# jixinya/EAMM

Hardware: AMD Instinct MI355X
Metric: 256x256 frames/sec (dense-motion + generator forward) (higher is better)
Workload: dtype f32; 1 GPU; 256x256, 10 keypoints, batch=16 synthetic frames per GPU per step, source encoded once per clip (BASELINE.json configs[2]); parallelism=frame-sharded x1

## Files before the change

eamm_amd/csrc/conv_winograd4.hip:

```cpp
#include "conv_common.h"

#include <algorithm>
#include <cstdlib>

namespace eamm {

typedef __attribute__((address_space(3))) void* lds_ptr_t;
typedef float f32x4_t __attribute__((ext_vector_type(4)));

template <int VEC> struct vec_of;
template <> struct vec_of<1> { typedef float type; };
template <> struct vec_of<2> { typedef float type __attribute__((ext_vector_type(2))); };
template <> struct vec_of<4> { typedef float type __attribute__((ext_vector_type(4))); };

template <typename T> __device__ __forceinline__ T vfma(float a, T x, T y);
template <> __device__ __forceinline__ float vfma<float>(float a, float x, float y) { return fmaf(a, x, y); }
template <> __device__ __forceinline__ vec_of<2>::type vfma(float a, vec_of<2>::type x, vec_of<2>::type y) {
    vec_of<2>::type r;
    r[0] = fmaf(a, x[0], y[0]); r[1] = fmaf(a, x[1], y[1]);
    return r;
}
template <> __device__ __forceinline__ vec_of<4>::type vfma(float a, vec_of<4>::type x, vec_of<4>::type y) {
    vec_of<4>::type r;
    r[0] = fmaf(a, x[0], y[0]); r[1] = fmaf(a, x[1], y[1]); r[2] = fmaf(a, x[2], y[2]); r[3] = fmaf(a, x[3], y[3]);
// ... 38 lines not shown
    const size_t total = Mq * cvn;
    const size_t bid = (by_xcd & 1) ? (size_t)xcd_remap((int)blockIdx.x, (int)gridDim.x) : (size_t)blockIdx.x;
    for (size_t idx = bid * blockDim.x + threadIdx.x; idx < total; idx += (size_t)gridDim.x * blockDim.x) {
        const int cv = (int)(idx % cvn);
        const size_t q = idx / cvn;
        const int qx = (int)(q % Wq);
        const int qy = (int)((q / Wq) % Hq);
        const int b = (int)(q / ((size_t)Wq * Hq));
        T sc = T(1.f), sh = T(0.f);
        if (s != nullptr) {
            sc = reinterpret_cast<const T*>(s)[cv];
            sh = reinterpret_cast<const T*>(t)[cv];
        }
        const T* img = reinterpret_cast<const T*>(x) + (size_t)b * H * W * cvn + cv;
        T d[6][6];
        int yo[6], xo[6];
        bool oky[6], okx[6];
#pragma unroll
        for (int i = 0; i < 6; ++i) {
            const int yy = 4 * qy - 1 + i, xx = 4 * qx - 1 + i;
            oky[i] = (unsigned)yy < (unsigned)H;
            okx[i] = (unsigned)xx < (unsigned)W;
            yo[i] = min(max(yy, 0), H - 1) * W;
            xo[i] = min(max(xx, 0), W - 1);
        }
#pragma unroll
        for (int i = 0; i < 6; ++i)
#pragma unroll
            for (int j = 0; j < 6; ++j) d[i][j] = img[(size_t)(yo[i] + xo[j]) * cvn];
#pragma unroll
        for (int i = 0; i < 6; ++i)
#pragma unroll
            for (int j = 0; j < 6; ++j) {
                T v = d[i][j];
                if (s != nullptr) v = vrelu_affine(v, sc, sh);
                d[i][j] = (oky[i] && okx[j]) ? v : T(0.f);
            }
#pragma unroll
        for (int j = 0; j < 6; ++j) bt6(d[0][j], d[1][j], d[2][j], d[3][j], d[4][j], d[5][j]);
        T* out = reinterpret_cast<T*>(V) + q * cvn + cv;
        const size_t plane = Mq * cvn;
#pragma unroll
        for (int i = 0; i < 6; ++i) {
            bt6(d[i][0], d[i][1], d[i][2], d[i][3], d[i][4], d[i][5]);
            if constexpr (VEC == 4) {
                if (by_xcd & 2) {
                    const __amdgpu_buffer_rsrc_t rs = __builtin_amdgcn_make_buffer_rsrc((void*)V, 0, (unsigned)(36 * plane * 16), 0x00020000);
#pragma unroll
                    for (int j = 0; j < 6; ++j)
                        __builtin_amdgcn_raw_buffer_store_b128(__builtin_bit_cast(u32x4, d[i][j]), rs,
                                                               (unsigned)(((size_t)(i * 6 + j) * plane + q * cvn + cv) * 16), 0, 2);
                    continue;
                }
            }
#pragma unroll
            for (int j = 0; j < 6; ++j) out[(size_t)(i * 6 + j) * plane] = d[i][j];
        }
    }
}

struct Wino4Args {
    const float* V;
    const float* U;
    const float* bias;
    unsigned v_bytes, u_bytes;
    int Mq, C, Cout;
    int H, W;
    int mtiles, ntiles;
    int act;
    const float* resid;
    float* out;
    int groups;
    float* zout;
    float* epi_scratch;
};

__constant__ float WINO4_AT[4][8] = {{1.f, 1.f, 1.f, 1.f, 1.f, 0.f, 0.f, 0.f},
                                     {0.f, 1.f, -1.f, 2.f, -2.f, 0.f, 0.f, 0.f},
                                     {0.f, 1.f, 1.f, 4.f, 4.f, 0.f, 0.f, 0.f},
                                     {0.f, 1.f, -1.f, 8.f, -8.f, 1.f, 0.f, 0.f}};

template <int NT, int WM, int WN, int SUB, int NST, int PE, int DBG = 0>
__global__ __launch_bounds__(WM* WN * 64) void wino4_gemm_kernel(const Wino4Args p) {
    constexpr int NW = WM * WN, NTHR = NW * 64;
    constexpr int BM = WM * 16, BN = WN * NT * 16, BK = CONV_BK;
    constexpr int A_STAGE = SUB * BM * BK, B_STAGE = SUB * BN * BK;
    constexpr int A_INSTR = BM / 8 / NW, B_INSTR = BN / 8 / NW;
    constexpr int NPIECE = SUB * (A_INSTR + B_INSTR);
    constexpr bool TRACE = DBG == 8 || DBG == 9;
    static_assert(BM % (8 * NW) == 0 && BN % (8 * NW) == 0, "tile rows must split evenly over the waves");
    static_assert(BK == 32, "two 16-wide K steps per chunk");

    extern __shared__ __attribute__((aligned(16))) float smem[];
    float* const As = smem;
    float* const Bs = smem + NST * A_STAGE;

    const int tid = threadIdx.x;
    const int lane = tid & 63;
    const int wave = __builtin_amdgcn_readfirstlane(tid >> 6);
    const int r16 = lane & 15, g = lane >> 4;
    const int wm = wave / WN, wn = wave % WN;

    const int L = xcd_remap(blockIdx.x, gridDim.x);
    const int ntile = L % p.ntiles;
    const int mtile = (L / p.ntiles) % p.mtiles;
    const int grp = L / (p.ntiles * p.mtiles);
    const int xis_per = 36 / p.groups;
    const int xi0 = grp * xis_per;
    const int mbase = mtile * BM;
    const int cchunks = p.C / BK;
    const int ci_base = xi0 * cchunks;
    const int nsuper = xis_per * cchunks / SUB;

    unsigned arow_off[A_INSTR];
#pragma unroll
    for (int j = 0; j < A_INSTR; ++j) {
        const int row = (wave * A_INSTR + j) * 8 + (lane >> 3);
        const int slot = (lane & 7) ^ ((row >> 1) & 7);
        const int m = mbase + row;
        arow_off[j] = m < p.Mq ? (unsigned)(m * p.C + slot * 4) * 4u : 0xFFFFF000u;
    }
    const unsigned b_lane = (unsigned)lane * 16u;
    const __amdgpu_buffer_rsrc_t rsv = __builtin_amdgcn_make_buffer_rsrc((void*)p.V, 0, p.v_bytes, 0x00020000);
    const __amdgpu_buffer_rsrc_t rsu = __builtin_amdgcn_make_buffer_rsrc((void*)p.U, 0, p.u_bytes, 0x00020000);
    const unsigned plane_bytes = (unsigned)p.Mq * (unsigned)p.C * 4u;
    const unsigned a_wrap = plane_bytes - (unsigned)(cchunks * BK * 4);

    unsigned sa_off = (unsigned)xi0 * plane_bytes;
    unsigned sb_off = (unsigned)((ntile * 36 * cchunks + ci_base) * BN * BK) * 4u +
                      (unsigned)(wave * B_INSTR * 8 * BK) * 4u;
    int dma_cc = 0, n_st = 0;
    auto dma_advance = [&]() {
        dma_cc += SUB;
        sa_off += SUB * BK * 4;
        if (dma_cc == cchunks) {
            dma_cc = 0;
            sa_off += a_wrap;
        }
        sb_off += SUB * BN * BK * 4;
        n_st = n_st + 1 == NST ? 0 : n_st + 1;
    };
    auto dma_piece = [&](auto kc) {
        constexpr int k = decltype(kc)::value;
        constexpr int sub = k / (A_INSTR + B_INSTR), r = k % (A_INSTR + B_INSTR);
        if constexpr (r < A_INSTR) {
            float* dst = As + n_st * A_STAGE + sub * (BM * BK) + (wave * A_INSTR + r) * (8 * BK) - sub * BK;
            const unsigned vo = arow_off[r];
            __builtin_amdgcn_raw_ptr_buffer_load_lds(rsv, (lds_ptr_t)dst, 16, vo, sa_off, sub * BK * 4, DBG == 40 ? 2 : 0);
        } else {
            constexpr int j = r - A_INSTR;
            float* dst = Bs + n_st * B_STAGE + sub * (BN * BK) + (wave * B_INSTR + j) * (8 * BK);
            __builtin_amdgcn_raw_ptr_buffer_load_lds(rsu, (lds_ptr_t)dst, 16, b_lane,
                                                     sb_off + (unsigned)((sub * BN + j * 8) * BK * 4), 0, 0);
        }
    };

    f32x4_t acc[NT];
    f32x4_t Z[4][NT];
    f32x4_t Y[16][NT];
    static_for<NT>([&](auto jc) {
        constexpr int j = decltype(jc)::value;
        static_for<4>([&](auto rc) {
            constexpr int r = decltype(rc)::value;
            acc[j][r] = 0.f;
            static_for<4>([&](auto qc) { Z[decltype(qc)::value][j][r] = 0.f; });
            static_for<16>([&](auto pc) { Y[decltype(pc)::value][j][r] = 0.f; });
        });
    });

    const int sw = (r16 >> 1) & 7;
    constexpr int STEPS = SUB * 2;
    constexpr int MF = 4 * NT;
    constexpr int TOTAL_MF = STEPS * MF;
    static_assert(PE >= 1 && NPIECE * PE <= TOTAL_MF, "DMA pieces must fit in the interval");
    auto compute = [&](int st, auto more_c, auto young_c) {
        constexpr bool MORE = decltype(more_c)::value && DBG != 1 && DBG != 9, YOUNG = decltype(young_c)::value;
        f32x4_t a[2], b[2][NT];
        auto fetch = [&](int step, int buf) {
            const int sub = step >> 1, s = step & 1;
            const int slot = ((4 * s + g) ^ sw) << 2;
            const float* a_base = As + st * A_STAGE + sub * (BM * BK) + (wm * 16 + r16) * BK + slot;
            const float* b_base = Bs + st * B_STAGE + sub * (BN * BK) + (wn * NT * 16 + r16) * BK + slot;
            a[buf] = *reinterpret_cast<const f32x4_t*>(a_base);
#pragma unroll
            for (int j = 0; j < NT; ++j) b[buf][j] = *reinterpret_cast<const f32x4_t*>(b_base + j * 16 * BK);
        };
        fetch(0, 0);
        if constexpr (MORE && YOUNG) static_for<NPIECE>([&](auto kc) { dma_piece(kc); });
        static_for<STEPS>([&](auto sc) {
            constexpr int step = decltype(sc)::value;
            if constexpr (step + 1 < STEPS) fetch(step + 1, (step + 1) & 1);
            __builtin_amdgcn_sched_barrier(0);
            static_for<MF>([&](auto qc) {
                constexpr int q = decltype(qc)::value;
                constexpr int t = q / NT, j = q % NT;
                acc[j] = __builtin_amdgcn_mfma_f32_16x16x4f32(a[step & 1][t], b[step & 1][j][t], acc[j], 0, 0, 0);
                constexpr int gi = step * MF + q;
                if constexpr (MORE && !YOUNG && gi % PE == PE - 1 && gi / PE < NPIECE) {
                    __builtin_amdgcn_sched_barrier(0);
                    dma_piece(std::integral_constant<int, gi / PE>{});
                    __builtin_amdgcn_sched_barrier(0);
                }
            });
        });
    };
    const bool young = wave >= NW / 2;
    auto interval = [&](int st, bool more) {
        if (more) {
            if (young) compute(st, std::true_type{}, std::true_type{});
            else compute(st, std::true_type{}, std::false_type{});
            dma_advance();
        } else {
            compute(st, std::false_type{}, std::false_type{});
        }
    };

    auto fold_x = [&](int j) {
        const float c0 = WINO4_AT[0][j], c1 = WINO4_AT[1][j], c2 = WINO4_AT[2][j], c3 = WINO4_AT[3][j];
        static_for<NT>([&](auto jc) {
            constexpr int jj = decltype(jc)::value;
            static_for<4>([&](auto rc) {
                constexpr int r = decltype(rc)::value;
                const float m = acc[jj][r];
                Z[0][jj][r] = fmaf(c0, m, Z[0][jj][r]);
                Z[1][jj][r] = fmaf(c1, m, Z[1][jj][r]);
                Z[2][jj][r] = fmaf(c2, m, Z[2][jj][r]);
                Z[3][jj][r] = fmaf(c3, m, Z[3][jj][r]);
                acc[jj][r] = 0.f;
            });
        });
    };
    auto fold_y = [&](int i) {
        const float c0 = WINO4_AT[0][i], c1 = WINO4_AT[1][i], c2 = WINO4_AT[2][i], c3 = WINO4_AT[3][i];
        static_for<NT>([&](auto jc) {
            constexpr int jj = decltype(jc)::value;
            static_for<4>([&](auto qc) {
                constexpr int q = decltype(qc)::value;
                static_for<4>([&](auto rc) {
                    constexpr int r = decltype(rc)::value;
                    const float z = Z[q][jj][r];
                    Y[0 + q][jj][r] = fmaf(c0, z, Y[0 + q][jj][r]);
                    Y[4 + q][jj][r] = fmaf(c1, z, Y[4 + q][jj][r]);
                    Y[8 + q][jj][r] = fmaf(c2, z, Y[8 + q][jj][r]);
                    Y[12 + q][jj][r] = fmaf(c3, z, Y[12 + q][jj][r]);
                    Z[q][jj][r] = 0.f;
                });
            });
        });
    };

    auto store_z = [&](int i) {
        static_for<4>([&](auto qc) {
            constexpr int q = decltype(qc)::value;
            static_for<NT>([&](auto jc) {
                constexpr int jj = decltype(jc)::value;
                const int col = ntile * BN + wn * NT * 16 + jj * 16 + r16;
                static_for<4>([&](auto rc) {
                    constexpr int r = decltype(rc)::value;
                    const int row = mbase + wm * 16 + 4 * g + r;
                    if (row < p.Mq && col < p.Cout) p.zout[((size_t)(i * 4 + q) * p.Mq + row) * p.Cout + col] = Z[q][jj][r];
                    Z[q][jj][r] = 0.f;
                });
            });
        });
    };

    constexpr int D = NST - 1;
    const int per_xi = cchunks / SUB;
    for (int k = 0; k < D && k < nsuper; ++k) {
        static_for<NPIECE>([&](auto kc) { dma_piece(kc); });
        dma_advance();
    }
    if (D > 1 && nsuper >= D) {
        asm volatile("s_waitcnt vmcnt(%0)" ::"n"((D - 1) * NPIECE) : "memory");
    } else {
        asm volatile("s_waitcnt vmcnt(0)" ::: "memory");
    }
    __syncthreads();
    int st = 0;
    int xi_left = per_xi, xj = xi0 % 6, xrow = xi0 / 6;
    const bool half_rows = p.groups == 12;
    for (int sc = 0; sc < nsuper; ++sc) {
        const bool more = sc + D < nsuper;
        long long ts0 = 0, ts1 = 0, ts2 = 0;
        if constexpr (TRACE) ts0 = __builtin_readcyclecounter();
        interval(st, more);
        if constexpr (TRACE) ts1 = __builtin_readcyclecounter();
        if (--xi_left == 0) {
            xi_left = per_xi;
            fold_x(xj);
            if (++xj == 6) {
                xj = 0;
                if (p.zout != nullptr)
                    store_z(half_rows ? grp : xrow++);
                else
                    fold_y(xrow++);
            }
        }
        if constexpr (TRACE) ts2 = __builtin_readcyclecounter();
        if (D > 1 && more) {
            asm volatile("s_waitcnt vmcnt(%0)" ::"n"((D - 1) * NPIECE) : "memory");
        } else {
            asm volatile("s_waitcnt vmcnt(0)" ::: "memory");
        }
        if constexpr (TRACE) {
            const long long ts3 = __builtin_readcyclecounter();
            if (blockIdx.x == 0 && lane == 0 && sc < 72) {
                long long* dbg = reinterpret_cast<long long*>(const_cast<float*>(p.resid)) + (wave * 72 + sc) * 4;
                dbg[0] = ts0; dbg[1] = ts1; dbg[2] = ts2; dbg[3] = ts3;
            }
        }
        __syncthreads();
        st = st + 1 == NST ? 0 : st + 1;
    }

    if (p.zout != nullptr) {
        if (half_rows && xj != 0) store_z(grp);
        return;
    }
    constexpr int LDO = BN + 4, C4 = BN / 4, RPP = NTHR / (4 * C4), PER = BM / RPP;
    static_assert(NTHR % (4 * C4) == 0 && BM % RPP == 0, "tile must split evenly over the threads");
    const int Hq = p.H >> 2, Wq = p.W >> 2;
    float bias[NT];
#pragma unroll
    for (int j = 0; j < NT; ++j) bias[j] = p.bias[ntile * BN + wn * NT * 16 + j * 16 + r16];
    const int e_c4 = tid % C4, e_px = (tid / C4) & 3, e_row0 = tid / (4 * C4);
    const int e_n = ntile * BN + e_c4 * 4;
    unsigned e_off[PER];
#pragma unroll
    for (int k = 0; k < PER; ++k) {
        const int m = mbase + e_row0 + k * RPP;
        const int qx = m % Wq, tq = m / Wq;
        const int qy = tq % Hq, bb = tq / Hq;
        const unsigned o = (unsigned)(((bb * p.H + 4 * qy) * p.W + 4 * qx + e_px) * p.Cout + e_n) * 4u;
        e_off[k] = (m < p.Mq && e_n < p.Cout) ? o : 0xFFFFFFF0u;
    }
    const unsigned out_bytes = (unsigned)p.Mq * 16u * (unsigned)p.Cout * 4u;
    const __amdgpu_buffer_rsrc_t rso = __builtin_amdgcn_make_buffer_rsrc((void*)p.out, 0, out_bytes, 0x00020000);
    const __amdgpu_buffer_rsrc_t rsr =
        __builtin_amdgcn_make_buffer_rsrc((void*)p.resid, 0, (p.resid != nullptr && !TRACE) ? out_bytes : 0u, 0x00020000);
    const float lo = p.act == ACT_RELU ? 0.f : -INFINITY;
    const unsigned row_bytes = (unsigned)p.W * (unsigned)p.Cout * 4u;
    const float* e_src = smem + (e_px * BM + e_row0) * LDO + e_c4 * 4;
    static_for<4>([&](auto pyc) {
        constexpr int py = decltype(pyc)::value;
        if (py) __syncthreads();
        static_for<4>([&](auto pxc) {
            constexpr int px = decltype(pxc)::value;
            static_for<NT>([&](auto jc) {
                constexpr int j = decltype(jc)::value;
                float* dst = smem + (px * BM + wm * 16 + 4 * g) * LDO + wn * NT * 16 + j * 16 + r16;
                static_for<4>([&](auto rc) {
                    constexpr int r = decltype(rc)::value;
                    dst[r * LDO] = Y[py * 4 + px][j][r] + bias[j];
                });
            });
        });
        __syncthreads();
        const unsigned soff = py * row_bytes;
        u32x4 rr[PER];
#pragma unroll
        for (int k = 0; k < PER; ++k) rr[k] = __builtin_amdgcn_raw_buffer_load_b128(rsr, e_off[k], soff, 0);
#pragma unroll
        for (int k = 0; k < PER; ++k) {
            f32x4_t v = *reinterpret_cast<const f32x4_t*>(e_src + k * RPP * LDO);
            const f32x4_t r4 = __builtin_bit_cast(f32x4_t, rr[k]);
            v = v + r4;
            v[0] = fmaxf(v[0], lo); v[1] = fmaxf(v[1], lo); v[2] = fmaxf(v[2], lo); v[3] = fmaxf(v[3], lo);
            __builtin_amdgcn_raw_buffer_store_b128(__builtin_bit_cast(u32x4, v), rso, e_off[k], soff, 0);
            if constexpr (DBG == 30) {
                const __amdgpu_buffer_rsrc_t rse = __builtin_amdgcn_make_buffer_rsrc((void*)p.epi_scratch, 0, 3u * out_bytes, 0x00020000);
                constexpr int extra = py == 3 ? 3 : 2;
                static_for<extra>([&](auto jc) {
                    __builtin_amdgcn_raw_buffer_store_b128(__builtin_bit_cast(u32x4, v), rse, e_off[k], soff + decltype(jc)::value * out_bytes, 0);
                });
            }
        }
    });
}

template <bool POOL, bool RESID>
__global__ __launch_bounds__(256) void wino4_output_transform_kernel(const float* __restrict__ Z, const float* __restrict__ bias,
                                                                     const float* __restrict__ resid, int Mq, int Cout, int H,
                                                                     int W, int act, float* __restrict__ out) {
    const int c4n = Cout >> 2;
    const int Hq = H >> 2, Wq = W >> 2;
    const size_t total = (size_t)Mq * c4n;
    const size_t plane = (size_t)Mq * c4n;
    for (size_t idx = (size_t)blockIdx.x * blockDim.x + threadIdx.x; idx < total; idx += (size_t)gridDim.x * blockDim.x) {
        const int c4 = (int)(idx % c4n);
        const int m = (int)(idx / c4n);
        const int qx = m % Wq, tq = m / Wq;
        const int qy = tq % Hq, b = tq / Hq;
        const f32x4_t* z = reinterpret_cast<const f32x4_t*>(Z) + idx;
        const f32x4_t bs = reinterpret_cast<const f32x4_t*>(bias)[c4];
        const float lo = act == ACT_RELU ? 0.f : -INFINITY;
        f32x4_t colsum[2];
#pragma unroll
        for (int q = 0; q < 4; ++q) {
            f32x4_t zi[6];
#pragma unroll
            for (int i = 0; i < 6; ++i) zi[i] = z[(size_t)(i * 4 + q) * plane];
            const f32x4_t s12 = zi[1] + zi[2], d12 = zi[1] - zi[2], s34 = zi[3] + zi[4], d34 = zi[3] - zi[4];
            f32x4_t y[4];
            y[0] = zi[0] + s12 + s34;
            y[1] = d12 + 2.f * d34;
            y[2] = s12 + 4.f * s34;
            y[3] = d12 + 8.f * d34 + zi[5];
            f32x4_t r4[4];
            if constexpr (RESID) {
#pragma unroll
                for (int pp = 0; pp < 4; ++pp)
                    r4[pp] = reinterpret_cast<const f32x4_t*>(resid)[(((size_t)(b * H + 4 * qy + pp) * W + 4 * qx + q) * Cout) / 4 + c4];
            }
#pragma unroll
            for (int pp = 0; pp < 4; ++pp) {
                f32x4_t v = y[pp] + bs;
                if constexpr (!POOL) {
                    const size_t o = (((size_t)(b * H + 4 * qy + pp) * W + 4 * qx + q) * Cout) / 4 + c4;
                    if constexpr (RESID) v = v + r4[pp];
                    v[0] = fmaxf(v[0], lo); v[1] = fmaxf(v[1], lo); v[2] = fmaxf(v[2], lo); v[3] = fmaxf(v[3], lo);
                    reinterpret_cast<f32x4_t*>(out)[o] = v;
                } else {
                    v[0] = fmaxf(v[0], lo); v[1] = fmaxf(v[1], lo); v[2] = fmaxf(v[2], lo); v[3] = fmaxf(v[3], lo);
                    y[pp] = v;
                }
            }
            if constexpr (POOL) {
                if ((q & 1) == 0) {
                    colsum[0] = y[0] + y[1];
                    colsum[1] = y[2] + y[3];
                } else {
#pragma unroll
                    for (int py = 0; py < 2; ++py) {
                        const f32x4_t v = 0.25f * (colsum[py] + (y[2 * py] + y[2 * py + 1]));
                        const size_t o = (((size_t)(b * (H >> 1) + 2 * qy + py) * (W >> 1) + 2 * qx + (q >> 1)) * Cout) / 4 + c4;
                        reinterpret_cast<f32x4_t*>(out)[o] = v;
                    }
                }
            }
        }
    }
}

void wino4_pack_host(const float* w, int Cout, int Cin, int BN, float* dst) {
    static const double G[6][3] = {{1.0 / 4, 0, 0},           {-1.0 / 6, -1.0 / 6, -1.0 / 6}, {-1.0 / 6, 1.0 / 6, -1.0 / 6},
                                   {1.0 / 24, 1.0 / 12, 1.0 / 6}, {1.0 / 24, -1.0 / 12, 1.0 / 6},  {0, 0, 1}};
    const int BK = CONV_BK, cch = Cin / BK;
    const int ntiles = (Cout + BN - 1) / BN;
    const size_t total = (size_t)ntiles * 36 * cch * BN * BK;
    for (size_t i = 0; i < total; ++i) dst[i] = 0.f;
    for (int o = 0; o < Cout; ++o) {
        const int nt = o / BN, nl = o % BN;
        for (int c = 0; c < Cin; ++c) {
            const float* gw = w + ((size_t)o * Cin + c) * 9;
            double tmp[6][3];
            for (int i = 0; i < 6; ++i)
                for (int k = 0; k < 3; ++k)
                    tmp[i][k] = G[i][0] * gw[0 * 3 + k] + G[i][1] * gw[1 * 3 + k] + G[i][2] * gw[2 * 3 + k];
            const int cc = c / BK, kl = c % BK;
            const int kk = ((((kl >> 2) ^ ((nl >> 1) & 7)) << 2) | (kl & 3));
            for (int i = 0; i < 6; ++i)
                for (int j = 0; j < 6; ++j) {
                    const double u = tmp[i][0] * G[j][0] + tmp[i][1] * G[j][1] + tmp[i][2] * G[j][2];
                    const int xi = i * 6 + j;
                    dst[(((size_t)nt * 36 * cch + (size_t)xi * cch + cc) * BN + nl) * BK + kk] = (float)u;
                }
        }
    }
}

size_t wino4_packed_elems(int Cout, int Cin, int BN) {
    return (size_t)((Cout + BN - 1) / BN) * 36 * (Cin / CONV_BK) * BN * CONV_BK;
}

hipError_t wino4_transform_launch(const float* x, const float* s, const float* t, int B, int H, int W, int C, float* V,
                                  hipStream_t stream) {
    if ((H & 3) || (W & 3) || (C & 3)) return hipErrorInvalidValue;
    static const int vec_env = [] {
        const int v = (int)knob_int("EAMM_WINO4_TR_VEC", 0);
        return (v == 1 || v == 2 || v == 4) ? v : 0;
    }();
    const int vec = vec_env ? vec_env : ((size_t)B * (H / 4) * (W / 4) * (C / 4) <= 64 * 256 ? 1 : 4);
    const size_t total = (size_t)B * (H / 4) * (W / 4) * (C / vec);
    const int blocks = (int)std::min<size_t>((total + 255) / 256, (size_t)1 << 20);
    static const int xcd = (int)knob_int("EAMM_WINO4_TR_XCD", 3);
    const int remap = ((size_t)blocks * 256 >= total ? (xcd & 1) : 0) | ((36.0 * total * 16 < 4.0e9 && vec == 4) ? (xcd & 2) : 0);
    if (vec == 1)
        hipLaunchKernelGGL(wino4_input_transform_kernel<1>, dim3(blocks), dim3(256), 0, stream, x, s, t, B, H, W, C, V, remap);
    else if (vec == 2)
        hipLaunchKernelGGL(wino4_input_transform_kernel<2>, dim3(blocks), dim3(256), 0, stream, x, s, t, B, H, W, C, V, remap);
    else
        hipLaunchKernelGGL(wino4_input_transform_kernel<4>, dim3(blocks), dim3(256), 0, stream, x, s, t, B, H, W, C, V, remap);
    return hipGetLastError();
}

template <int SUB, int NST, int PE, int DBG = 0, int WM = 4>
static hipError_t wino4_launch_variant(const Wino4Args& a, hipStream_t stream) {
    constexpr int NT = 2, WN = 2;
    constexpr int BM = WM * 16, BN = WN * NT * 16;
    constexpr size_t lds_loop = sizeof(float) * NST * SUB * (BM + BN) * CONV_BK;
    constexpr size_t lds_epi = sizeof(float) * 4 * BM * (BN + 4);
    constexpr size_t lds = lds_loop > lds_epi ? lds_loop : lds_epi;
    static_assert(lds <= 160 * 1024, "LDS budget");
    auto kern = wino4_gemm_kernel<NT, WM, WN, SUB, NST, PE, DBG>;
    static lds_once_mask configured{0};
    if (hipError_t e = ensure_dynamic_lds(kern, lds, &configured); e != hipSuccess) return e;
    note_mfma_flops(2.0 * 36.0 * a.mtiles * BM * (double)a.ntiles * BN * a.C);
    hipLaunchKernelGGL(kern, dim3(a.mtiles * a.ntiles * a.groups), dim3(WM * WN * 64), lds, stream, a);
    return hipGetLastError();
}

hipError_t wino4_gemm_launch(const WinoLayer& L, const float* V, int B, int H, int W, int act, const float* resid,
                             float* out, hipStream_t stream, int variant, int groups, float* zbuf, int pool) {
    constexpr int BM = 64, BN = 64;
    if (pool && (groups == 1 || resid != nullptr)) return hipErrorInvalidValue;
    if (L.tile != 4 || L.BN != BN || (L.Cout & 3) || L.Cin % (2 * CONV_BK) || (H & 3) || (W & 3))
        return hipErrorInvalidValue;
    Wino4Args a{};
    a.V = V;
    a.U = L.u;
    a.bias = L.bias;
    a.Mq = B * (H / 4) * (W / 4);
    a.C = L.Cin;
    a.Cout = L.Cout;
    a.H = H;
    a.W = W;
    a.mtiles = (a.Mq + BM - 1) / BM;
    a.ntiles = L.ntiles;
    static const int narrow_max = (int)knob_int("EAMM_WINO4_NARROW_MAX_BLOCKS", 128);
    const bool narrow = groups == 6 && a.mtiles * a.ntiles * groups <= narrow_max && L.Cin % (4 * CONV_BK) == 0;
    if (narrow) a.mtiles = (a.Mq + 31) / 32;
    a.act = act;
    a.resid = resid;
    a.out = out;
    if (groups != 1 && groups != 2 && groups != 3 && groups != 6) return hipErrorInvalidValue;
    if (groups > 1 && zbuf == nullptr) return hipErrorInvalidValue;
    a.groups = groups;
    a.zout = groups > 1 ? zbuf : nullptr;
#ifdef EAMM_EXPERIMENTS
    a.epi_scratch = (variant == 50 && groups == 1) ? zbuf : nullptr;
    if (variant == 50 && a.epi_scratch == nullptr) variant = 3;
#else
    if (variant == 10 || variant == 16 || variant == 17 || variant == 50) return hipErrorInvalidValue;
#endif
    const size_t vb = (size_t)36 * a.Mq * a.C * sizeof(float), ub = wino4_packed_elems(L.Cout, L.Cin, BN) * sizeof(float);
    if (vb >= 0xFFFFF000ull || ub >= 0xFFFFF000ull) return hipErrorInvalidValue;
    a.v_bytes = (unsigned)vb;
    a.u_bytes = (unsigned)ub;
    const bool sub4 = L.Cin % (4 * CONV_BK) == 0;
    hipError_t e = hipErrorInvalidValue;
    if (narrow) variant = 30;
    switch (variant) {
        case 30: e = wino4_launch_variant<4, 2, 4, 0, 2>(a, stream); break;
#ifdef EAMM_EXPERIMENTS
        case 50: e = sub4 ? wino4_launch_variant<4, 2, 8, 30>(a, stream) : wino4_launch_variant<2, 2, 4>(a, stream); break;
        case 10: e = wino4_launch_variant<4, 2, 4, 1>(a, stream); break;
        case 16: e = wino4_launch_variant<4, 2, 4, 8>(a, stream); break;
        case 17: e = wino4_launch_variant<4, 2, 4, 9>(a, stream); break;
#endif
        case 0: e = sub4 ? wino4_launch_variant<4, 2, 4>(a, stream) : wino4_launch_variant<2, 2, 4>(a, stream); break;
        case 3: e = sub4 ? wino4_launch_variant<4, 2, 8>(a, stream) : wino4_launch_variant<2, 2, 4>(a, stream); break;
        case 6: e = sub4 ? wino4_launch_variant<4, 2, 8, 40>(a, stream) : wino4_launch_variant<2, 2, 4>(a, stream); break;
        default: break;
    }
    if (e != hipSuccess || groups == 1) return e;
    const size_t total = (size_t)a.Mq * (L.Cout / 4);
    const int blocks = (int)std::min<size_t>((total + 255) / 256, (size_t)1 << 20);
    if (pool)
        hipLaunchKernelGGL((wino4_output_transform_kernel<true, false>), dim3(blocks), dim3(256), 0, stream, zbuf, L.bias, resid,
                           a.Mq, L.Cout, H, W, act, out);
    else if (resid != nullptr)
        hipLaunchKernelGGL((wino4_output_transform_kernel<false, true>), dim3(blocks), dim3(256), 0, stream, zbuf, L.bias, resid,
                           a.Mq, L.Cout, H, W, act, out);
    else
        hipLaunchKernelGGL((wino4_output_transform_kernel<false, false>), dim3(blocks), dim3(256), 0, stream, zbuf, L.bias, resid,
                           a.Mq, L.Cout, H, W, act, out);
    return hipGetLastError();
}

}
```

eamm_amd/csrc/eamm_api.hip:

```cpp
#include "eamm_ctx.h"

namespace {

void expected_keys(const eamm_ctx* c, std::vector<std::string>* keys) {
    auto block = [&](const std::string& p) { block_keys(p, keys); };
    const std::string dm = "dense_motion_network.";
    for (int i = 0; i < c->nb; ++i) block(dm + "hourglass.encoder.down_blocks." + std::to_string(i));
    for (int i = 0; i < c->nb; ++i) block(dm + "hourglass.decoder.up_blocks." + std::to_string(i));
    if (c->nb > 0) {
        keys->push_back(dm + "mask.weight");
        keys->push_back(dm + "mask.bias");
        if (c->cfg.estimate_occlusion_map) {
            keys->push_back(dm + "occlusion.weight");
            keys->push_back(dm + "occlusion.bias");
        }
        if (c->cfg.dm_inv_scale != 1) keys->push_back(dm + "down.weight");
    }
    block("first");
    for (int i = 0; i < c->nd; ++i) block("down_blocks." + std::to_string(i));
    for (int i = 0; i < c->nd; ++i) block("up_blocks." + std::to_string(i));
    for (int i = 0; i < c->cfg.num_bottleneck_blocks; ++i) {
        const std::string r = "bottleneck.r" + std::to_string(i);
        for (const char* s : {".conv1.weight", ".conv1.bias", ".conv2.weight", ".conv2.bias", ".norm1.weight",
                              ".norm1.bias", ".norm1.running_mean", ".norm1.running_var", ".norm2.weight",
// ... 136 lines not shown
    if (g.num_down_blocks < 1 || g.num_bottleneck_blocks < 1)
        return fail(nullptr, EAMM_ERR_ARG, "need at least one down block and one bottleneck block");
    if (g.max_frames < 1 || g.max_sources < 1) return fail(nullptr, EAMM_ERR_ARG, "max_frames / max_sources < 1");
    const int div_g = 1 << g.num_down_blocks, div_m = has_dm ? g.dm_inv_scale << g.dm_num_blocks : 1;
    if (g.height % div_g || g.width % div_g || g.height % div_m || g.width % div_m)
        return fail(nullptr, EAMM_ERR_ARG, "frame %dx%d not divisible for %d down blocks / %d hourglass levels",
                    g.height, g.width, g.num_down_blocks, g.dm_num_blocks);
    {
        const double hw = (double)g.height * g.width, F = g.max_frames;
        const double biggest = std::max({F * hw * 32.0,
                                         F * hw * (double)round_up(g.block_expansion, 32),
                                         4.0 * F * (hw / (1 << (2 * g.num_down_blocks))) *
                                             round_up(std::min(g.max_features, g.block_expansion << g.num_down_blocks), 32)}) * 4.0;
        if (biggest >= 4294967280.0)
            return fail(nullptr, EAMM_ERR_ARG, "max_frames=%d at %dx%d needs a %.1f GiB activation tensor; the limit is 4 GiB "
                        "per tensor -- lower max_frames", g.max_frames, g.height, g.width, biggest / 1073741824.0);
    }
    {
        DeviceGuard probe(device);
        if (probe.status != hipSuccess) return fail(nullptr, EAMM_ERR_HIP, "hipSetDevice(%d) failed", device);
    }

    eamm_ctx* c = new eamm_ctx();
    c->cfg = g;
    c->device = device;
    c->H = g.height;
    c->W = g.width;
    if (!has_dm) c->cfg.dm_inv_scale = 1;
    c->h = c->H / c->cfg.dm_inv_scale;
    c->w = c->W / c->cfg.dm_inv_scale;
    c->nd = g.num_down_blocks;
    c->nb = g.dm_num_blocks;
    c->K = g.num_kp;
    c->hf = c->H >> c->nd;
    c->wf = c->W >> c->nd;
    c->Cimg = g.num_channels;
    c->G = c->Cimg > 3 ? 2 : 1;
    c->Cpl = 3 * c->G;
    c->Cp0 = round_up((c->K + 1) * 4 * c->G, 32);
    for (int i = 0; i < c->nb; ++i) c->enc_r.push_back(std::min(g.dm_max_features, g.dm_block_expansion << (i + 1)));
    for (int i = c->nb - 1; i >= 0; --i) c->dec_r.push_back(std::min(g.dm_max_features, g.dm_block_expansion << i));
    c->down_r.push_back(g.block_expansion);
    for (int i = 0; i < c->nd; ++i) c->down_r.push_back(std::min(g.max_features, g.block_expansion << (i + 1)));
    for (int i = 0; i < c->nd; ++i) c->up_r.push_back(std::min(g.max_features, g.block_expansion << (c->nd - i - 1)));
    c->Cb_r = c->down_r.back();
    auto pad32 = [&](const std::vector<int>& r, std::vector<int>* p) {
        for (int v : r) {
            p->push_back(round_up(v, 32));
            c->padded_widths |= p->back() != v;
        }
    };
    pad32(c->enc_r, &c->enc_c);
    pad32(c->dec_r, &c->dec_c);
    pad32(c->down_r, &c->down_c);
    pad32(c->up_r, &c->up_c);
    c->Cb = c->down_c.back();
    read_tile_knobs(c);
    c->wino_min_m = env_int("EAMM_WINO_MIN_M", c->wino_min_m);
    c->wino4_min_m = env_int("EAMM_WINO4_MIN_M", c->wino4_min_m);
    c->wino_tile = env_int("EAMM_WINO_TILE", c->wino_tile);
    c->col7 = env_int("EAMM_COL7", c->col7);
    c->final_fused = env_int("EAMM_FINAL_FUSED", c->final_fused);
    c->final_fused_min_rows = env_int("EAMM_FINAL_FUSED_MIN_ROWS", c->final_fused_min_rows);
    c->bneck_chains = env_int("EAMM_BNECK_CHAINS", c->bneck_chains);
    c->pass_chains = env_int("EAMM_PASS_CHAINS", c->pass_chains);
    c->pass_chains = c->pass_chains < 0 ? 1 : std::min(c->pass_chains, 4);
    c->bneck_chains = std::max(1, std::min(c->bneck_chains, 16));
    c->warp_joint = env_int("EAMM_WARP_JOINT", c->warp_joint);
    c->wino4_variant = env_int("EAMM_WINO4_VARIANT", c->wino4_variant);
    c->wino4_variant_pinned = getenv("EAMM_WINO4_VARIANT") != nullptr;
    {
        int cus = 0;
        if (hipDeviceGetAttribute(&cus, hipDeviceAttributeMultiprocessorCount, device) == hipSuccess && cus > 0) c->cus = cus;
        else (void)hipGetLastError();
    }
#ifdef EAMM_EXPERIMENTS
    c->epi_v = env_int("EAMM_WINO4_EPI_V", c->epi_v);
#else
    for (const char* bad : {"EAMM_WINO4_EPI_V", "EAMM_COL7_DBG"})
        if (getenv(bad) && atoi(getenv(bad)) != 0) {
            delete c;
            return fail(nullptr, EAMM_ERR_ARG, "%s is a wrong-results timing experiment: it needs a library built with make EXPERIMENTS=1", bad);
        }
    if (c->wino4_variant == 10 || c->wino4_variant == 16 || c->wino4_variant == 17 || c->wino4_variant == 50) {
        const int v = c->wino4_variant;
        delete c;
        return fail(nullptr, EAMM_ERR_ARG, "EAMM_WINO4_VARIANT=%d is a wrong-results timing experiment: it needs make EXPERIMENTS=1", v);
    }
    if (c->wino4_variant != 0 && c->wino4_variant != 3 && c->wino4_variant != 6) {
        const int v = c->wino4_variant;
        delete c;
        return fail(nullptr, EAMM_ERR_ARG, "EAMM_WINO4_VARIANT=%d: the F(4x4) GEMM has the pipeline variants 0, 3 and 6", v);
    }
#endif
    c->pass_chains_min_frames = env_int("EAMM_PASS_CHAINS_MIN_FRAMES", c->pass_chains_min_frames);
    c->pass_chains_min_blocks = env_int("EAMM_PASS_CHAINS_MIN_BLOCKS", c->pass_chains_min_blocks);
    c->head_col7_min_tiles = env_int("EAMM_HEAD_COL7_MIN_TILES", c->head_col7_min_tiles);
    c->enc_wino = env_int("EAMM_ENC_WINO", c->enc_wino);
    c->first7 = env_int("EAMM_FIRST7", c->first7);
    c->enc_wino_min_mflop = env_int("EAMM_ENC_WINO_MIN_MFLOP", c->enc_wino_min_mflop);
    c->enc_wino_min_tiles = env_int("EAMM_ENC_WINO_MIN_TILES", c->enc_wino_min_tiles);
    c->dma_cfg_n256 = env_int("EAMM_DMA_CFG_N256", c->dma_cfg_n256);
    c->dma_cfg_n128 = env_int("EAMM_DMA_CFG_N128", c->dma_cfg_n128);
    c->dma_cfg_n64 = env_int("EAMM_DMA_CFG_N64", c->dma_cfg_n64);
    *out = c;
    return EAMM_OK;
}

void eamm_destroy(eamm_ctx* c) {
    if (!c) return;
    DeviceGuard guard(c->device);
    free_owned(c);
    for (auto& e : c->prof_events) (void)hipEventDestroy(e);
    for (auto& e : c->prof_chain_ev) (void)hipEventDestroy(e);
    if (c->ev_fork) (void)hipEventDestroy(c->ev_fork);
    if (c->ev_warp) (void)hipEventDestroy(c->ev_warp);
    for (auto& e : c->ev_join) (void)hipEventDestroy(e);
    for (auto& st : c->own_streams) (void)hipStreamDestroy(st);
    delete c;
}

int eamm_load_tensor(eamm_ctx* c, const char* key, const float* host, const int64_t* shape, int ndim) {
    return store_tensor(c, key, host, shape, ndim);
}

int eamm_finalize_weights(eamm_ctx* c) {
    if (!c) return EAMM_ERR_ARG;
    if (c->finalized) return fail(c, EAMM_ERR_STATE, "weights already finalised");
    DeviceGuard guard(c->device);
    if (guard.status != hipSuccess) return fail(c, EAMM_ERR_HIP, "hipSetDevice(%d) failed", c->device);
    const eamm_config& g = c->cfg;
    {
        std::vector<std::string> want;
        expected_keys(c, &want);
        if (int krc = check_keys(c, want)) return krc;
    }
    if (c->padded_widths || c->Cimg != 3) {
        if (c->train_mode)
            return fail(c, EAMM_ERR_ARG, "a training-mode handle needs three image channels and channel widths that are multiples of 32 "
                        "(its BatchNorm kernels read the module's own statistics tensors); the module takes the operator composition "
                        "for such a generator");
        if (int prc = pad_state_dict(c)) return prc;
    }
    const std::string dm = "dense_motion_network.";
    int rc;
    const bool tr = c->train_mode;
    auto nm = [&](const std::string& norm) { return tr ? std::string() : norm; };
    c->hg_enc.resize(c->nb);
    const int cin0 = (c->K + 1) * 4 * c->G;
    for (int i = 0; i < c->nb; ++i) {
        const std::string p = dm + "hourglass.encoder.down_blocks." + std::to_string(i);
        const int cr = i == 0 ? cin0 : c->enc_c[i - 1], cp = i == 0 ? c->Cp0 : c->enc_c[i - 1];
        if ((rc = build_set(c, {{p + ".conv", nm(p + ".norm")}}, cr, cp, 0, 0, &c->hg_enc[i], MODE_PLAIN))) return rc;
    }
    c->hg_dec.resize(c->nb);
    for (int i = 0; i < c->nb; ++i) {
        const std::string p = dm + "hourglass.decoder.up_blocks." + std::to_string(i);
        const int c0 = i == 0 ? c->enc_c[c->nb - 1] : c->dec_c[i - 1];
        const int c1 = i == 0 ? 0 : c->enc_c[c->nb - 1 - i];
        if ((rc = build_set(c, {{p + ".conv", nm(p + ".norm")}}, c0, c0, c1, c1, &c->hg_dec[i], MODE_PHASE))) return rc;
    }
    if (c->nb > 0) {
        std::vector<FoldSpec> parts = {{dm + "mask", ""}};
        if (g.estimate_occlusion_map) parts.push_back({dm + "occlusion", ""});
        const int nc = c->K + 1 + (g.estimate_occlusion_map ? 1 : 0);
        if (7 * nc <= 128 && env_int("EAMM_HEAD_ROWSPLIT", 1)) {
            std::vector<float> hb;
// ... 371 lines not shown
```

Baseline: 4039 frames/s.

## Overlap Winograd F(4x4) epilogue output stores with the final GEMM intervals

Moves the output-transform epilogue of the fused Winograd GEMM into the main K loop. Once the first five output row-folds are complete, each wave stages finished output planes through a small per-wave LDS area and writes them out (bias, residual, ReLU) while later intervals still compute. This replaces the end-of-kernel block-wide LDS transpose and its syncthreads. It also skips the unneeded FMAs in the last row fold and adds a variant-60 experiment that disables the epilogue. In exchange it adds a per-wave staging buffer to the LDS footprint, extra residual loads inside the pipelined loop, and more complex control flow.

New measurement: 3975 frames/s. -1.6%, worse.

```diff
diff --git a/eamm_amd/csrc/conv_winograd4.hip b/eamm_amd/csrc/conv_winograd4.hip
--- a/eamm_amd/csrc/conv_winograd4.hip
+++ b/eamm_amd/csrc/conv_winograd4.hip
@@ -144,12 +144,15 @@
 
 template <int NT, int WM, int WN, int SUB, int NST, int PE, int DBG = 0>
 __global__ __launch_bounds__(WM* WN * 64) void wino4_gemm_kernel(const Wino4Args p) {
-    constexpr int NW = WM * WN, NTHR = NW * 64;
+    constexpr int NW = WM * WN;
     constexpr int BM = WM * 16, BN = WN * NT * 16, BK = CONV_BK;
     constexpr int A_STAGE = SUB * BM * BK, B_STAGE = SUB * BN * BK;
     constexpr int A_INSTR = BM / 8 / NW, B_INSTR = BN / 8 / NW;
     constexpr int NPIECE = SUB * (A_INSTR + B_INSTR);
     constexpr bool TRACE = DBG == 8 || DBG == 9;
+    constexpr int RING = NST * (A_STAGE + B_STAGE);
+    constexpr int WSTG = 4 * (4 * NT * 16 + 16);
+    static_assert(NT == 2, "the staging layout below is for rows of 32 floats");
     static_assert(BM % (8 * NW) == 0 && BN % (8 * NW) == 0, "tile rows must split evenly over the waves");
     static_assert(BK == 32, "two 16-wide K steps per chunk");
 
@@ -192,7 +195,7 @@
     unsigned sb_off = (unsigned)((ntile * 36 * cchunks + ci_base) * BN * BK) * 4u +
                       (unsigned)(wave * B_INSTR * 8 * BK) * 4u;
     int dma_cc = 0, n_st = 0;
-    auto dma_advance = [&]() {
+    auto dma_advance = [&]() __attribute__((always_inline)) {
         dma_cc += SUB;
         sa_off += SUB * BK * 4;
         if (dma_cc == cchunks) {
@@ -202,7 +205,7 @@
         sb_off += SUB * BN * BK * 4;
         n_st = n_st + 1 == NST ? 0 : n_st + 1;
     };
-    auto dma_piece = [&](auto kc) {
+    auto dma_piece = [&](auto kc) __attribute__((always_inline)) {
         constexpr int k = decltype(kc)::value;
         constexpr int sub = k / (A_INSTR + B_INSTR), r = k % (A_INSTR + B_INSTR);
         if constexpr (r < A_INSTR) {
@@ -235,10 +238,10 @@
     constexpr int MF = 4 * NT;
     constexpr int TOTAL_MF = STEPS * MF;
     static_assert(PE >= 1 && NPIECE * PE <= TOTAL_MF, "DMA pieces must fit in the interval");
-    auto compute = [&](int st, auto more_c, auto young_c) {
+    auto compute = [&](int st, auto more_c, auto young_c) __attribute__((always_inline)) {
         constexpr bool MORE = decltype(more_c)::value && DBG != 1 && DBG != 9, YOUNG = decltype(young_c)::value;
         f32x4_t a[2], b[2][NT];
-        auto fetch = [&](int step, int buf) {
+        auto fetch = [&](int step, int buf) __attribute__((always_inline)) {
             const int sub = step >> 1, s = step & 1;
             const int slot = ((4 * s + g) ^ sw) << 2;
             const float* a_base = As + st * A_STAGE + sub * (BM * BK) + (wm * 16 + r16) * BK + slot;
@@ -267,7 +270,7 @@
         });
     };
     const bool young = wave >= NW / 2;
-    auto interval = [&](int st, bool more) {
+    auto interval = [&](int st, bool more) __attribute__((always_inline)) {
         if (more) {
             if (young) compute(st, std::true_type{}, std::true_type{});
             else compute(st, std::true_type{}, std::false_type{});
@@ -277,7 +280,7 @@
         }
     };
 
-    auto fold_x = [&](int j) {
+    auto fold_x = [&](int j) __attribute__((always_inline)) {
         const float c0 = WINO4_AT[0][j], c1 = WINO4_AT[1][j], c2 = WINO4_AT[2][j], c3 = WINO4_AT[3][j];
         static_for<NT>([&](auto jc) {
             constexpr int jj = decltype(jc)::value;
@@ -292,7 +295,8 @@
             });
         });
     };
-    auto fold_y = [&](int i) {
+    auto fold_y = [&](int i, auto last_c) __attribute__((always_inline)) {
+        constexpr bool LAST = decltype(last_c)::value;
         const float c0 = WINO4_AT[0][i], c1 = WINO4_AT[1][i], c2 = WINO4_AT[2][i], c3 = WINO4_AT[3][i];
         static_for<NT>([&](auto jc) {
             constexpr int jj = decltype(jc)::value;
@@ -301,9 +305,11 @@
                 static_for<4>([&](auto rc) {
                     constexpr int r = decltype(rc)::value;
                     const float z = Z[q][jj][r];
-                    Y[0 + q][jj][r] = fmaf(c0, z, Y[0 + q][jj][r]);
-                    Y[4 + q][jj][r] = fmaf(c1, z, Y[4 + q][jj][r]);
-                    Y[8 + q][jj][r] = fmaf(c2, z, Y[8 + q][jj][r]);
+                    if constexpr (!LAST) {
+                        Y[0 + q][jj][r] = fmaf(c0, z, Y[0 + q][jj][r]);
+                        Y[4 + q][jj][r] = fmaf(c1, z, Y[4 + q][jj][r]);
+                        Y[8 + q][jj][r] = fmaf(c2, z, Y[8 + q][jj][r]);
+                    }
                     Y[12 + q][jj][r] = fmaf(c3, z, Y[12 + q][jj][r]);
                     Z[q][jj][r] = 0.f;
                 });
@@ -311,7 +317,7 @@
         });
     };
 
-    auto store_z = [&](int i) {
+    auto store_z = [&](int i) __attribute__((always_inline)) {
         static_for<4>([&](auto qc) {
             constexpr int q = decltype(qc)::value;
             static_for<NT>([&](auto jc) {
@@ -333,6 +339,87 @@
         static_for<NPIECE>([&](auto kc) { dma_piece(kc); });
         dma_advance();
     }
+
+    constexpr bool EPI = DBG != 60;
+    const bool fused = WM == 4 && p.zout == nullptr;
+    float* const stg = smem + RING + wave * (WSTG + NT * 16);
+    const int Hq = p.H >> 2, Wq = p.W >> 2;
+    unsigned e_off[NT];
+    const unsigned out_bytes = (unsigned)p.Mq * 16u * (unsigned)p.Cout * 4u;
+    const unsigned row_bytes = (unsigned)p.W * (unsigned)p.Cout * 4u, px_bytes = (unsigned)p.Cout * 4u;
+    const __amdgpu_buffer_rsrc_t rso = __builtin_amdgcn_make_buffer_rsrc((void*)p.out, 0, fused ? out_bytes : 0u, 0x00020000);
+    const __amdgpu_buffer_rsrc_t rsr =
+        __builtin_amdgcn_make_buffer_rsrc((void*)p.resid, 0, (fused && p.resid != nullptr && !TRACE) ? out_bytes : 0u, 0x00020000);
+    const float lo = p.act == ACT_RELU ? 0.f : -INFINITY;
+    {
+        const int e_n = ntile * BN + wn * NT * 16 + (lane & 7) * 4;
+#pragma unroll
+        for (int j = 0; j < NT; ++j) {
+            if (g == 0) stg[WSTG + j * 16 + r16] = p.bias[ntile * BN + wn * NT * 16 + j * 16 + r16];
+            const int row = (lane >> 3) + 8 * j;
+            const int m = mbase + wm * 16 + row;
+            const int qx = m % Wq, tq = m / Wq;
+            const int qy = tq % Hq, bb = tq / Hq;
+            const unsigned o = (unsigned)(((bb * p.H + 4 * qy) * p.W + 4 * qx) * p.Cout + e_n) * 4u;
+            e_off[j] = (m < p.Mq && e_n < p.Cout) ? o : 0xFFFFFFF0u;
+        }
+    }
+    auto plane_soff = [&](int m) __attribute__((always_inline)) { return (unsigned)(m >> 2) * row_bytes + (unsigned)(m & 3) * px_bytes; };
+    auto resid_load = [&](int m, u32x4(&rr)[NT]) __attribute__((always_inline)) {
+        const unsigned soff = plane_soff(m);
+#pragma unroll
+        for (int k = 0; k < NT; ++k) {
+            const unsigned vo = e_off[k];
+            rr[k] = __builtin_amdgcn_raw_buffer_load_b128(rsr, vo, soff, 0);
+        }
+    };
+    auto stage = [&](auto mc) __attribute__((always_inline)) {
+        constexpr int m = decltype(mc)::value;
+        int l = lane;
+        asm volatile("" : "+v"(l));
+        float* const stg_w = stg + (l >> 4) * 144 + (l & 15);
+        static_for<NT>([&](auto jc) {
+            constexpr int j = decltype(jc)::value;
+            static_for<4>([&](auto rc) {
+                constexpr int r = decltype(rc)::value;
+                stg_w[r * 32 + j * 16] = Y[m][j][r];
+            });
+        });
+        asm volatile("; plane %0 staged" ::"n"(m) : "memory");
+    };
+    auto stage_rt = [&](int m) __attribute__((always_inline)) {
+        static_for<12>([&](auto mc) {
+            if (m == decltype(mc)::value) stage(mc);
+        });
+    };
+    auto emit = [&](int m, const u32x4(&rr)[NT]) __attribute__((always_inline)) {
+        int l = lane;
+        asm volatile("" : "+v"(l));
+        const float* const stg_r = stg + (l >> 5) * 144 + ((l >> 3) & 3) * 32 + (l & 7) * 4;
+        const f32x4_t bias4 = *reinterpret_cast<const f32x4_t*>(stg + WSTG + (l & 7) * 4);
+        __builtin_amdgcn_wave_barrier();
+        const unsigned soff = plane_soff(m);
+#pragma unroll
+        for (int k = 0; k < NT; ++k) {
+            f32x4_t v = *reinterpret_cast<const f32x4_t*>(stg_r + k * 288) + bias4;
+            v = v + __builtin_bit_cast(f32x4_t, rr[k]);
+            v[0] = fmaxf(v[0], lo); v[1] = fmaxf(v[1], lo); v[2] = fmaxf(v[2], lo); v[3] = fmaxf(v[3], lo);
+            const unsigned vo = e_off[k];
+            __builtin_amdgcn_raw_buffer_store_b128(__builtin_bit_cast(u32x4, v), rso, vo, soff, 0);
+            if constexpr (DBG == 30) {
+                const __amdgpu_buffer_rsrc_t rse = __builtin_amdgcn_make_buffer_rsrc((void*)p.epi_scratch, 0, 3u * out_bytes, 0x00020000);
+                const int extra = (m >> 2) == 3 ? 3 : 2;
+                for (int x = 0; x < extra; ++x)
+                    __builtin_amdgcn_raw_buffer_store_b128(__builtin_bit_cast(u32x4, v), rse, vo, soff + x * out_bytes, 0);
+            }
+        }
+        __builtin_amdgcn_wave_barrier();
+    };
+    const int n_row = 6 * per_xi;
+    const int sc_early = (fused && EPI) ? nsuper - n_row - 1 : nsuper;
+    int credit = 0, n_staged = 0;
+    u32x4 rr[2][NT];
+
     if (D > 1 && nsuper >= D) {
         asm volatile("s_waitcnt vmcnt(%0)" ::"n"((D - 1) * NPIECE) : "memory");
     } else {
@@ -346,6 +433,18 @@
         const bool more = sc + D < nsuper;
         long long ts0 = 0, ts1 = 0, ts2 = 0;
         if constexpr (TRACE) ts0 = __builtin_readcyclecounter();
+        int nw = 0;
+        if (sc >= sc_early) {
+            if (sc + 1 < nsuper) {
+                credit += 12;
+                if (credit > 0) { ++nw; credit -= n_row; }
+                if (credit > 0) { ++nw; credit -= n_row; }
+                if (nw >= 1) resid_load(n_staged, rr[0]);
+            } else {
+                resid_load(12, rr[0]);
+                resid_load(13, rr[1]);
+            }
+        }
         interval(st, more);
         if constexpr (TRACE) ts1 = __builtin_readcyclecounter();
         if (--xi_left == 0) {
@@ -355,16 +454,24 @@
                 xj = 0;
                 if (p.zout != nullptr)
                     store_z(half_rows ? grp : xrow++);
-                else
-                    fold_y(xrow++);
+                else if (xrow < 5)
+                    fold_y(xrow++, std::false_type{});
             }
         }
         if constexpr (TRACE) ts2 = __builtin_readcyclecounter();
+        if (nw >= 1) stage_rt(n_staged);
         if (D > 1 && more) {
             asm volatile("s_waitcnt vmcnt(%0)" ::"n"((D - 1) * NPIECE) : "memory");
         } else {
             asm volatile("s_waitcnt vmcnt(0)" ::: "memory");
         }
+        if (nw >= 1) emit(n_staged, rr[0]);
+        if (nw == 2) {
+            resid_load(n_staged + 1, rr[1]);
+            stage_rt(n_staged + 1);
+            emit(n_staged + 1, rr[1]);
+        }
+        n_staged += nw;
         if constexpr (TRACE) {
             const long long ts3 = __builtin_readcyclecounter();
             if (blockIdx.x == 0 && lane == 0 && sc < 72) {
@@ -376,69 +483,30 @@
         st = st + 1 == NST ? 0 : st + 1;
     }
 
-    if (p.zout != nullptr) {
+    if (!fused) {
         if (half_rows && xj != 0) store_z(grp);
         return;
     }
-    constexpr int LDO = BN + 4, C4 = BN / 4, RPP = NTHR / (4 * C4), PER = BM / RPP;
-    static_assert(NTHR % (4 * C4) == 0 && BM % RPP == 0, "tile must split evenly over the threads");
-    const int Hq = p.H >> 2, Wq = p.W >> 2;
-    float bias[NT];
-#pragma unroll
-    for (int j = 0; j < NT; ++j) bias[j] = p.bias[ntile * BN + wn * NT * 16 + j * 16 + r16];
-    const int e_c4 = tid % C4, e_px = (tid / C4) & 3, e_row0 = tid / (4 * C4);
-    const int e_n = ntile * BN + e_c4 * 4;
-    unsigned e_off[PER];
-#pragma unroll
-    for (int k = 0; k < PER; ++k) {
-        const int m = mbase + e_row0 + k * RPP;
-        const int qx = m % Wq, tq = m / Wq;
-        const int qy = tq % Hq, bb = tq / Hq;
-        const unsigned o = (unsigned)(((bb * p.H + 4 * qy) * p.W + 4 * qx + e_px) * p.Cout + e_n) * 4u;
-        e_off[k] = (m < p.Mq && e_n < p.Cout) ? o : 0xFFFFFFF0u;
-    }
-    const unsigned out_bytes = (unsigned)p.Mq * 16u * (unsigned)p.Cout * 4u;
-    const __amdgpu_buffer_rsrc_t rso = __builtin_amdgcn_make_buffer_rsrc((void*)p.out, 0, out_bytes, 0x00020000);
-    const __amdgpu_buffer_rsrc_t rsr =
-        __builtin_amdgcn_make_buffer_rsrc((void*)p.resid, 0, (p.resid != nullptr && !TRACE) ? out_bytes : 0u, 0x00020000);
-    const float lo = p.act == ACT_RELU ? 0.f : -INFINITY;
-    const unsigned row_bytes = (unsigned)p.W * (unsigned)p.Cout * 4u;
-    const float* e_src = smem + (e_px * BM + e_row0) * LDO + e_c4 * 4;
-    static_for<4>([&](auto pyc) {
-        constexpr int py = decltype(pyc)::value;
-        if (py) __syncthreads();
-        static_for<4>([&](auto pxc) {
-            constexpr int px = decltype(pxc)::value;
-            static_for<NT>([&](auto jc) {
-                constexpr int j = decltype(jc)::value;
-                float* dst = smem + (px * BM + wm * 16 + 4 * g) * LDO + wn * NT * 16 + j * 16 + r16;
-                static_for<4>([&](auto rc) {
-                    constexpr int r = decltype(rc)::value;
-                    dst[r * LDO] = Y[py * 4 + px][j][r] + bias[j];
-                });
-            });
+    if constexpr (!EPI) {
+        if (p.Mq >= 0) return;
+        rr[0][0] = rr[0][1] = u32x4{0u, 0u, 0u, 0u};
+        static_for<12>([&](auto mc) {
+            stage(mc);
+            emit(decltype(mc)::value, rr[0]);
         });
-        __syncthreads();
-        const unsigned soff = py * row_bytes;
-        u32x4 rr[PER];
-#pragma unroll
-        for (int k = 0; k < PER; ++k) rr[k] = __builtin_amdgcn_raw_buffer_load_b128(rsr, e_off[k], soff, 0);
-#pragma unroll
-        for (int k = 0; k < PER; ++k) {
-            f32x4_t v = *reinterpret_cast<const f32x4_t*>(e_src + k * RPP * LDO);
-            const f32x4_t r4 = __builtin_bit_cast(f32x4_t, rr[k]);
-            v = v + r4;
-            v[0] = fmaxf(v[0], lo); v[1] = fmaxf(v[1], lo); v[2] = fmaxf(v[2], lo); v[3] = fmaxf(v[3], lo);
-            __builtin_amdgcn_raw_buffer_store_b128(__builtin_bit_cast(u32x4, v), rso, e_off[k], soff, 0);
-            if constexpr (DBG == 30) {
-                const __amdgpu_buffer_rsrc_t rse = __builtin_amdgcn_make_buffer_rsrc((void*)p.epi_scratch, 0, 3u * out_bytes, 0x00020000);
-                constexpr int extra = py == 3 ? 3 : 2;
-                static_for<extra>([&](auto jc) {
-                    __builtin_amdgcn_raw_buffer_store_b128(__builtin_bit_cast(u32x4, v), rse, e_off[k], soff + decltype(jc)::value * out_bytes, 0);
-                });
-            }
-        }
-    });
+    }
+    u32x4 rr2[2][NT];
+    resid_load(14, rr2[0]);
+    resid_load(15, rr2[1]);
+    fold_y(5, std::true_type{});
+    stage(std::integral_constant<int, 12>{});
+    emit(12, rr[0]);
+    stage(std::integral_constant<int, 13>{});
+    emit(13, rr[1]);
+    stage(std::integral_constant<int, 14>{});
+    emit(14, rr2[0]);
+    stage(std::integral_constant<int, 15>{});
+    emit(15, rr2[1]);
 }
 
 template <bool POOL, bool RESID>
@@ -561,9 +629,7 @@
 static hipError_t wino4_launch_variant(const Wino4Args& a, hipStream_t stream) {
     constexpr int NT = 2, WN = 2;
     constexpr int BM = WM * 16, BN = WN * NT * 16;
-    constexpr size_t lds_loop = sizeof(float) * NST * SUB * (BM + BN) * CONV_BK;
-    constexpr size_t lds_epi = sizeof(float) * 4 * BM * (BN + 4);
-    constexpr size_t lds = lds_loop > lds_epi ? lds_loop : lds_epi;
+    constexpr size_t lds = sizeof(float) * (NST * SUB * (BM + BN) * CONV_BK + WM * WN * (576 + 32));
     static_assert(lds <= 160 * 1024, "LDS budget");
     auto kern = wino4_gemm_kernel<NT, WM, WN, SUB, NST, PE, DBG>;
     static lds_once_mask configured{0};
@@ -604,7 +670,7 @@
     a.epi_scratch = (variant == 50 && groups == 1) ? zbuf : nullptr;
     if (variant == 50 && a.epi_scratch == nullptr) variant = 3;
 #else
-    if (variant == 10 || variant == 16 || variant == 17 || variant == 50) return hipErrorInvalidValue;
+    if (variant == 10 || variant == 16 || variant == 17 || variant == 50 || variant == 60) return hipErrorInvalidValue;
 #endif
     const size_t vb = (size_t)36 * a.Mq * a.C * sizeof(float), ub = wino4_packed_elems(L.Cout, L.Cin, BN) * sizeof(float);
     if (vb >= 0xFFFFF000ull || ub >= 0xFFFFF000ull) return hipErrorInvalidValue;
@@ -620,6 +686,7 @@
         case 10: e = wino4_launch_variant<4, 2, 4, 1>(a, stream); break;
         case 16: e = wino4_launch_variant<4, 2, 4, 8>(a, stream); break;
         case 17: e = wino4_launch_variant<4, 2, 4, 9>(a, stream); break;
+        case 60: e = sub4 ? wino4_launch_variant<4, 2, 8, 60>(a, stream) : wino4_launch_variant<2, 2, 4, 60>(a, stream); break;
 #endif
         case 0: e = sub4 ? wino4_launch_variant<4, 2, 4>(a, stream) : wino4_launch_variant<2, 2, 4>(a, stream); break;
         case 3: e = sub4 ? wino4_launch_variant<4, 2, 8>(a, stream) : wino4_launch_variant<2, 2, 4>(a, stream); break;
diff --git a/eamm_amd/csrc/eamm_api.hip b/eamm_amd/csrc/eamm_api.hip
--- a/eamm_amd/csrc/eamm_api.hip
+++ b/eamm_amd/csrc/eamm_api.hip
@@ -242,7 +242,7 @@
             delete c;
             return fail(nullptr, EAMM_ERR_ARG, "%s is a wrong-results timing experiment: it needs a library built with make EXPERIMENTS=1", bad);
         }
-    if (c->wino4_variant == 10 || c->wino4_variant == 16 || c->wino4_variant == 17 || c->wino4_variant == 50) {
+    if (c->wino4_variant == 10 || c->wino4_variant == 16 || c->wino4_variant == 17 || c->wino4_variant == 50 || c->wino4_variant == 60) {
         const int v = c->wino4_variant;
         delete c;
         return fail(nullptr, EAMM_ERR_ARG, "EAMM_WINO4_VARIANT=%d is a wrong-results timing experiment: it needs make EXPERIMENTS=1", v);
```
